# f1tenth/f1tenth_gym

Measured on AMD Instinct MI355X. Metric: agent-steps/s (1080-beam scan + ST dynamics), higher is better.
Workload: dtype f64

## Files before the change

f1tenth_gym_amd/csrc/f110_hip.hip:

```cpp
#include <hip/hip_runtime.h>
#include <rccl/rccl.h>

#include <dlfcn.h>

#include <algorithm>
#include <chrono>
#include <cmath>
#include <cstdarg>
#include <cstdio>
#include <cstdlib>
#include <cstring>
#include <map>
#include <mutex>
#include <new>
#include <set>
#include <string>
#include <vector>

#include "../../include/f110.h"
#include "f110_kernels.hpp"



#ifdef F110_EXPERIMENTAL
constexpr bool kExperimental = true;
#else
constexpr bool kExperimental = false;
#endif

struct ExpSwitches {
    int scan_flat = 0;
    int long_prio = 0;
    int scan_occupancy = 0;
    int scan_env_counter = 0;
    int integrate_duo = -1;
    int group_split = 0;
    int integrate_fan = -1;
    int tiny_general_tail = 0;
    int tiny_start_probe = 0;
    long probe_calls = 0;
    double probe_us[3] = {0, 0, 0};
    uint64_t tiny_trace = 0;
    uint64_t scan_trace = 0;
};

struct f110_sim {
    f110_config cfg{};
    int N = 0;
    hipStream_t stream = nullptr;
    hipStream_t side_stream = nullptr;
    hipEvent_t ev_integrated = nullptr, ev_collided = nullptr;
    AgentArrays dev{};
    ScanConst k{};
    bool has_map = false;
    uint32_t step_magic = 0, step_shift = 0;
    int scan_tasks_per_wave = 1, num_cus = 256;
    bool scan_tasks_auto = false;
    double ttc_side_max = INFINITY, ttc_cos_max = INFINITY;
    int dir_stride = 0;
    int scan_block = 64;
    double *d_params_all = nullptr;
    double *d_params = nullptr, *d_noise = nullptr, *d_scan_angles = nullptr, *d_beam_cos = nullptr, *d_side = nullptr;
    struct MapSlot {
        double *d_dt_row = nullptr, *d_dt_pad = nullptr;
        ScanConst k{};
        uint8_t *d_occ = nullptr;
    };
    std::vector<MapSlot> extra_maps;
    MapFast *d_maps_fast = nullptr;
    ScanConst *d_maps_full = nullptr;
    int32_t *d_env_map = nullptr;
    uint32_t *d_scan_order = nullptr;
    bool multi_map = false;
    ScanConst *d_k = nullptr;
    ScanConst k_uploaded{};
    unsigned long long *d_path_stats = nullptr;
    bool path_stats_on = false;
    double *d_dt_row = nullptr, *d_dt_pad = nullptr, *d_actions = nullptr, *d_poses = nullptr;
    double2 *d_cs = nullptr;
    uint8_t *d_mask = nullptr;
    int groups = 1;
    std::vector<hipStream_t> gstreams;
    std::vector<hipStream_t> gowned;
    std::vector<hipEvent_t> gevents;
    hipEvent_t ev_main = nullptr;
    bool groups_auto = true;
    bool touched = true;
    int last_blocks = 0;
    int group_probes = 0;
    bool groups_busy = false;
    bool main_dirty = true;
    NoiseGen noise_gen{};
    uint64_t *d_zig_k = nullptr;
    double *d_zig_w = nullptr, *d_zig_f = nullptr;
    U128 *d_jump = nullptr;
    U128 *d_rng_state = nullptr, *d_rng_seed = nullptr, *d_rng_rowstate = nullptr;
    int noise_rows_ready = 0;
    int noise_rows_alloc = 0;
    hipStream_t noise_stream = nullptr;
    hipEvent_t ev_noise = nullptr, ev_noise_src = nullptr;
    bool noise_ahead = false;
    int noise_ahead_upto = 0, noise_ahead_alloc = 0;
    double *noise_ahead_block = nullptr;
    std::vector<double *> noise_retired;
    long long noise_ub = 0;
    int noise_src = 0;
    uint64_t noise_src_id[4] = {0, 0, 0, 0};
    void *d_state_blob = nullptr;
    size_t state_blob_bytes = 0;
    unsigned long long *d_lookups = nullptr;
    bool lookups_on = false;
    int collide_mode = 0;
    bool task_order = false;
    uint32_t *d_tflags[2] = {nullptr, nullptr}, *d_tlist[2] = {nullptr, nullptr}, *d_tcount = nullptr;
    TaskSched tsched[2]{};
    bool sched_allocated = false;
    uint32_t task_cap_alloc = 0;
    uint32_t task_epoch = 2, task_cap = 0, task_thr = 96;
    uint32_t task_cap_div = 32, task_rev = 0;
    ExpSwitches exp;
    uint32_t *d_env_done = nullptr;
// ... 13 lines not shown
    EpisodeArrays ep{};
    bool has_episode = false;
    double *d_rot_stage = nullptr;
    void *d_packed = nullptr;
    bool hb_valid = false;
    f110_host_block hb_host{};
    HostBlock hb_dev{};
    const double *hb_actions_host = nullptr, *hb_actions_dev = nullptr;
    bool hb_scans_by_kernel = false;
    unsigned long long *hb_seq_host = nullptr;
    unsigned int *hb_blocks_done = nullptr;
    unsigned long long hb_seq = 0;
    double hs_enqueue_us = 0, hs_wait_us = 0;
    FusedHost *d_fused = nullptr;
    FusedHost fused_host_copy{};
    bool fused_valid = false;
    long long hs_calls = 0;
    TinyCtl tiny{};
    void *tiny_mem = nullptr;
    int tiny_off = 0;
    int last_launches = 0;
    struct TrackSlot {
        double *d_cols = nullptr;
        double *d_pts = nullptr;
        double *d_attr = nullptr;
        int32_t nattr = 0;
        int32_t nseg = 0, closed = 0, npts = 0;
        double L = 0.0;
    };
    std::vector<TrackSlot> tracks;
    TrackDesc *d_tracks = nullptr;
    PreviewAttr *d_track_attrs = nullptr;
    int n_tracks_dev = 0;
    bool tracks_dirty = true;
    bool track_lds = false;
    bool track_on = false, track_checked = false;
    std::vector<int32_t> env_map_host;
    double *d_trk = nullptr;
    int32_t *d_trk_seg = nullptr;
    double *d_trk_cache = nullptr;
    int32_t *d_trk_ok = nullptr;
    f110_track_host trk_pinned{};
    HostBlock trk_hb{};
    bool trk_pinned_on = false;
    const float *obs_pinned = nullptr;
    const float *preview_pinned = nullptr;
    const float *neighbors_pinned = nullptr;
    const float *rollout_pinned = nullptr;
    double *d_roll_end = nullptr;
    size_t roll_end_cap = 0;
    GapSpec *d_gap_specs = nullptr;
    int32_t *d_gap_assign = nullptr;
    int gap_specs = 0, gap_max_w = 0;
    uint8_t *d_occ0 = nullptr;
    std::vector<RenderSlot> render_slots;
    RenderSlot *d_render_slots = nullptr;
    size_t render_slots_cap = 0;
    RenderFrame *d_render_frames = nullptr;
    size_t render_frames_cap = 0;
    RenderCar *d_render_cars = nullptr;
    int32_t *d_render_agents = nullptr;
    size_t render_agents_cap = 0;
    uint8_t *d_render_stage = nullptr;
    size_t render_stage_cap = 0;
    struct ResetSampler {
        bool on = false;
        SamplerJob job{};
    } rs;
    hipEvent_t ev_begin = nullptr, ev_end = nullptr;
    bool profiling = false;
    std::vector<hipEvent_t> prof_events;
    size_t prof_used = 0;
    char err[512] = {0};
};

struct StepRequest {
    bool tiny = false;
    const double *tiny_actions = nullptr;
    bool fuse = false;
    unsigned long long seq = 0;
    const HostBlock *hb = nullptr;
    int episode = 0, auto_reset = 0;
    bool defer_draw = false;
};

static thread_local char g_err[512] = {0};

static int fail(f110_sim *h, int code, const char *fmt, ...)
{
    char buf[512];
    va_list ap;
    va_start(ap, fmt);
    vsnprintf(buf, sizeof buf, fmt, ap);
    va_end(ap);
    snprintf(g_err, sizeof g_err, "%s", buf);
    if (h) snprintf(h->err, sizeof h->err, "%s", buf);
    return code;
}

#define HIPCHK(h, call)                                                                              \
    do {                                                                                             \
        hipError_t e_ = (call);                                                                      \
        if (e_ != hipSuccess)                                                                        \
            return fail(h, F110_ERR_HIP, "%s failed: %s (%s:%d)", #call, hipGetErrorString(e_), __FILE__, __LINE__); \
    } while (0)

template <typename T>
static int dmalloc(f110_sim *h, T **p, size_t count)
{
    HIPCHK(h, hipMalloc(reinterpret_cast<void **>(p), count * sizeof(T) > 0 ? count * sizeof(T) : 8));
    return F110_OK;
}

#define TRY(expr)              \
    do {                       \
        int rc_ = (expr);      \
        if (rc_ != F110_OK) return rc_; \
    } while (0)

static int join_groups(f110_sim *h)
{
    if (h->comm_inflight) {
        HIPCHK(h, hipStreamWaitEvent(h->stream, h->ev_gather_done[0], 0));
        HIPCHK(h, hipStreamWaitEvent(h->stream, h->ev_gather_done[1], 0));
        h->comm_inflight = false;
    }
    if (!h->groups_busy) return F110_OK;
    for (size_t g = 0; g < h->gstreams.size(); ++g) {
        if (h->gstreams[g] == h->stream) continue;
        HIPCHK(h, hipEventRecord(h->gevents[g], h->gstreams[g]));
        HIPCHK(h, hipStreamWaitEvent(h->stream, h->gevents[g], 0));
    }
    h->groups_busy = false;
    return F110_OK;
}

#define ENTER(h)                                          \
    do {                                                  \
        HIPCHK(h, hipSetDevice((h)->cfg.device_id));      \
        TRY(join_groups(h));                              \
        (h)->main_dirty = true;                           \
        (h)->touched = true;                              \
    } while (0)

static int track_invalidate(f110_sim *h);
static int track_prepare(f110_sim *h);
static int track_launch(f110_sim *h, hipStream_t st, int mode, int begin, int count);
static bool tiny_applies(const f110_sim *h);
static void noise_release(f110_sim *h);
static void sampler_release(f110_sim *h);
static int sampler_launch(f110_sim *h, hipStream_t st, int mode, int e0, int count, const uint8_t *d_mask, int ego);
static int step_submit(f110_sim *h, const double *d_actions, const StepRequest &rq, bool &host_written);

constexpr int kMaxEnvBlocks = 16;
struct EnvBlock { hipStream_t stream; int e0, count; };
static void gap_launch_armed(f110_sim *h, const EnvBlock &b, double *d_actions);
struct EnvBlocks {
    EnvBlock b[kMaxEnvBlocks];
    int n = 0;
    const EnvBlock *begin() const { return b; }
    const EnvBlock *end() const { return b + n; }
};

static int group_envs(const f110_sim *h)
{
    const int E = h->cfg.num_envs, G = h->groups;
// ... 136 lines not shown
}

static int task_order_setup(f110_sim *h, bool on)
{
    const size_t n_tasks = (size_t)h->N * (((size_t)h->cfg.num_beams + 63) / 64);
    if (!on || n_tasks >= 0x7fffffffu) {
        h->task_order = false;
        return F110_OK;
    }
    if (!h->sched_allocated) {
        h->task_cap_alloc = (uint32_t)std::max<size_t>(64, kExperimental ? n_tasks : n_tasks / h->task_cap_div);
        for (int q = 0; q < 2; ++q) {
            TRY(dmalloc(h, &h->d_tflags[q], n_tasks));
            TRY(dmalloc(h, &h->d_tlist[q], (size_t)h->task_cap_alloc));
            HIPCHK(h, hipMemsetAsync(h->d_tflags[q], 0, sizeof(uint32_t) * n_tasks, h->stream));
        }
        TRY(dmalloc(h, &h->d_tcount, 4));
        HIPCHK(h, hipMemsetAsync(h->d_tcount, 0, 4 * sizeof(uint32_t), h->stream));
        h->sched_allocated = true;
    }
    h->task_cap = std::min<uint32_t>(h->task_cap_alloc, (uint32_t)std::max<size_t>(64, n_tasks / h->task_cap_div));
    for (int q = 0; q < 2; ++q)
        h->tsched[q] = TaskSched{h->d_tflags[q ^ 1], h->d_tflags[q], h->d_tlist[q ^ 1], h->d_tlist[q], h->d_tcount + (q ^ 1), h->d_tcount + q, h->task_cap, h->task_thr, {nullptr, nullptr, nullptr, nullptr, nullptr, nullptr, nullptr, nullptr}, 0u, 0u};
    HIPCHK(h, hipStreamSynchronize(h->stream));
    h->task_order = true;
    return F110_OK;
}

extern "C" {

const char *f110_last_error(const f110_sim *h) { return (h && h->err[0]) ? h->err : g_err; }
int f110_abi_version(void) { return F110_ABI_VERSION; }

int f110_device_count(int *count)
{
    int n = 0;
    hipError_t e = hipGetDeviceCount(&n);
    if (e != hipSuccess) {
        if (count) *count = 0;
        return fail(nullptr, F110_ERR_HIP, "hipGetDeviceCount failed: %s", hipGetErrorString(e));
    }
    if (count) *count = n;
    return F110_OK;
}

int f110_device_pci_bus_id(int32_t device, char *out, int32_t len)
{
    if (!out || len < 16) return fail(nullptr, F110_ERR_INVALID, "f110_device_pci_bus_id: buffer of at least 16 bytes required");
    const hipError_t e = hipDeviceGetPCIBusId(out, len, device);
    if (e != hipSuccess) return fail(nullptr, F110_ERR_HIP, "hipDeviceGetPCIBusId(%d) failed: %s", device, hipGetErrorString(e));
    return F110_OK;
}

#ifndef F110_SRC_HASH
#define F110_SRC_HASH "unknown"
#endif
const char *f110_build_info(void) { return "csrc=" F110_SRC_HASH; }

int f110_is_experimental(void) { return kExperimental ? 1 : 0; }

int f110_exp_set(f110_sim *h, const char *key, int32_t value)
{
    if (!h || !key) return fail(h, F110_ERR_INVALID, "null argument");
    if (!kExperimental) return fail(h, F110_ERR_STATE, "f110_exp_set(%s) is available in the experimental build only (libf110_hip_exp.so)", key);
    ENTER(h);
    HIPCHK(h, hipStreamSynchronize(h->stream));
    const std::string k(key);
    if (k == "scan_flat") h->exp.scan_flat = value;
    else if (k == "long_prio") h->exp.long_prio = value;
    else if (k == "scan_occupancy") h->exp.scan_occupancy = value;
    else if (k == "scan_env_counter") h->exp.scan_env_counter = value;
    else if (k == "integrate_duo") h->exp.integrate_duo = value;
    else if (k == "integrate_fan") h->exp.integrate_fan = value;
    else if (k == "group_split") h->exp.group_split = value;
    else if (k == "step_tiny") h->tiny_off = value == 0 ? 1 : 0;
    else if (k == "tiny_start_probe") {
        if (!value && h->exp.tiny_start_probe && h->exp.probe_calls)
            std::fprintf(stderr, "[tiny_start_probe] %ld steps: call -> launched %.2f us, launched -> first wave seen %.2f us, first wave seen -> completion word seen %.2f us\n",
                         h->exp.probe_calls, h->exp.probe_us[0] / h->exp.probe_calls, h->exp.probe_us[1] / h->exp.probe_calls, h->exp.probe_us[2] / h->exp.probe_calls);
        h->exp.tiny_start_probe = value;
        h->exp.probe_calls = 0;
        h->exp.probe_us[0] = h->exp.probe_us[1] = h->exp.probe_us[2] = 0;
    }
    else if (k == "tiny_general_tail") h->exp.tiny_general_tail = value;
    else if (k == "tiny_trace_hi") h->exp.tiny_trace = (h->exp.tiny_trace & 0xffffffffull) | ((uint64_t)(uint32_t)value << 32);
    else if (k == "tiny_trace_lo") h->exp.tiny_trace = (h->exp.tiny_trace & ~0xffffffffull) | (uint64_t)(uint32_t)value;
    else if (k == "scan_trace_hi") h->exp.scan_trace = (h->exp.scan_trace & 0xffffffffull) | ((uint64_t)(uint32_t)value << 32);
    else if (k == "scan_trace_lo") h->exp.scan_trace = (h->exp.scan_trace & ~0xffffffffull) | (uint64_t)(uint32_t)value;
    else if (k == "collide_mode") {
        if (value < 0 || value > 3) return fail(h, F110_ERR_INVALID, "collide_mode must be 0..3");
        h->collide_mode = value;
    }
    else if (k == "task_order") return task_order_setup(h, value != 0);
    else if (k == "task_cap_div" || k == "task_rev") {
        if (k == "task_rev") h->task_rev = value != 0;
        else h->task_cap_div = (uint32_t)std::max(1, value);
        if (h->task_order) return task_order_setup(h, true);
    } else if (k == "task_thr") {
        h->task_thr = (uint32_t)value;
        if (h->task_order) return task_order_setup(h, true);
    }
    else if (k == "pad_tiled" || k == "scan_nt" || k == "finalize_wave" || k == "spec_from" || k == "scan_stream" || k == "stream_refill" || k == "stream_block" ||
             k == "stream_grid")
        return fail(h, F110_ERR_INVALID, "f110_exp_set: '%s' was retired in round 6 with the variant it switched (DESIGN.md section 8)", key);
    else
        return fail(h, F110_ERR_INVALID, "f110_exp_set: unknown key '%s'", key);
    return F110_OK;
}

static void default_beam_tables(const f110_config &c, std::vector<double> &sa, std::vector<double> &co, std::vector<double> &sd)
{
    const int B = c.num_beams;
    const double incr = c.fov / (B - 1);
    const double dist_sides = c.params[F110_P_WIDTH] / 2., dist_fr = (c.params[F110_P_LF] + c.params[F110_P_LR]) / 2.;
    sa.resize(B); co.resize(B); sd.resize(B);
    for (int i = 0; i < B; ++i) {
        const double angle = -c.fov / 2. + i * incr;
        double to_side, to_fr;
        sa[i] = angle;
        co[i] = std::cos(angle);
        if (angle > 0) {
            if (angle < kPi / 2) { to_side = dist_sides / std::sin(angle); to_fr = dist_fr / std::cos(angle); }
            else { to_side = dist_sides / std::cos(angle - kPi / 2.); to_fr = dist_fr / std::sin(angle - kPi / 2.); }
        } else {
            if (angle > -kPi / 2) { to_side = dist_sides / std::sin(-angle); to_fr = dist_fr / std::cos(-angle); }
            else { to_side = dist_sides / std::cos(-angle - kPi / 2); to_fr = dist_fr / std::sin(-angle - kPi / 2); }
        }
        sd[i] = to_side < to_fr ? to_side : to_fr;
    }
}

static hipError_t streams_concurrent(hipStream_t a, hipStream_t b, bool *yes)
{
    *yes = false;
    unsigned *d = nullptr, hres[2] = {0u, 0u};
    hipError_t e = hipMalloc(&d, 2 * sizeof(unsigned));
    if (e != hipSuccess) return e;
    do {
        if ((e = hipMemsetAsync(d, 0, 2 * sizeof(unsigned), a)) != hipSuccess) break;
        if ((e = hipStreamSynchronize(a)) != hipSuccess) break;
        if ((e = hipStreamSynchronize(b)) != hipSuccess) break;
        hipLaunchKernelGGL(k_probe_wait, dim3(1), dim3(1), 0, a, d, d + 1, 30000ull);
        hipLaunchKernelGGL(k_probe_set, dim3(1), dim3(1), 0, b, d);
        if ((e = hipStreamSynchronize(a)) != hipSuccess) break;
        if ((e = hipStreamSynchronize(b)) != hipSuccess) break;
        if ((e = hipMemcpy(hres, d, sizeof hres, hipMemcpyDeviceToHost)) != hipSuccess) break;
        *yes = hres[1] != 0u;
    } while (0);
    (void)hipFree(d);
    return e;
}

static std::mutex g_registry_mu;
static std::set<f110_sim *> g_handles;
static std::map<const char *, size_t> g_host_blocks;

int f110_create(const f110_config *cfg, f110_sim **out)
{
    if (!cfg || !out) return fail(nullptr, F110_ERR_INVALID, "f110_create: null argument");
    *out = nullptr;
    if (cfg->abi_version != F110_ABI_VERSION) return fail(nullptr, F110_ERR_INVALID, "ABI version mismatch (%d vs %d)", cfg->abi_version, F110_ABI_VERSION);
    if (cfg->num_envs < 1 || cfg->num_agents < 1 || cfg->num_beams < 2 || cfg->theta_dis < 2)
        return fail(nullptr, F110_ERR_INVALID, "f110_create: num_envs/num_agents >= 1, num_beams/theta_dis >= 2 required");
    if (cfg->integrator != F110_INTEGRATOR_RK4 && cfg->integrator != F110_INTEGRATOR_EULER)
        return fail(nullptr, F110_ERR_INVALID, "Invalid Integrator Specified. Please choose RK4 or Euler");
    if (cfg->map_layout == F110_MAP_TILED_F64 || cfg->map_layout == F110_MAP_CODE8 || cfg->map_layout == F110_MAP_WINDOW_LDS)
// ... 1958 lines not shown
#define DIRS_SCAN(PM, ID)                                                                                                                    \
    do {                                                                                                                                     \
        if (cnt) hipLaunchKernelGGL((k_scan_dirs_agent<PM, ID, true>), grid, block, 0, st, j, h->k, h->d_maps_fast, h->d_maps_full, tpa);     \
        else hipLaunchKernelGGL((k_scan_dirs_agent<PM, ID, false>), grid, block, 0, st, j, h->k, h->d_maps_fast, h->d_maps_full, tpa);        \
    } while (0)
            if (h->multi_map) DIRS_SCAN(true, false);
            else if (h->k.ident_rot) DIRS_SCAN(false, true);
            else DIRS_SCAN(false, false);
#undef DIRS_SCAN
            break;
        }
        case SCAN_AGENT_SCHED: {
            const uint32_t tpa = ((uint32_t)B + 63u) / 64u;
            agent_grid(tpa, grid, wpb, h->scan_tasks_per_wave);
            const uint32_t parity = h->task_epoch & 1u;
            j.sched = h->tsched[parity];
            j.epoch_r = h->task_epoch - 1u;
            j.epoch_w = h->task_epoch;
            j.long_blocks = (h->task_cap + wpb - 1) / wpb;
            j.long_prio = (uint32_t)h->exp.long_prio;
            j.long_rev = h->task_rev;
            h->task_epoch += 1u;
            const dim3 sgrid(grid.x + j.long_blocks);
            size_t slds = 0;
#ifdef F110_EXPERIMENTAL
            if (h->exp.scan_occupancy > 0 && h->scan_block == 64) slds = (size_t)(160 * 1024 / (4 * h->exp.scan_occupancy)) & ~(size_t)255;
#endif
            if (h->k.ident_rot)
                hipLaunchKernelGGL((k_scan_rays_agent<false, true, false, true>), sgrid, block, slds, st, j, h->k, h->d_maps_fast, h->d_maps_full, tpa);
            else
                hipLaunchKernelGGL((k_scan_rays_agent<false, false, false, true>), sgrid, block, slds, st, j, h->k, h->d_maps_fast, h->d_maps_full, tpa);
            break;
        }
        case SCAN_AGENT: {
            const uint32_t tpa = ((uint32_t)B + 63u) / 64u;
            agent_grid(tpa, grid, wpb, h->scan_tasks_per_wave);
            size_t lds = 0;
#ifdef F110_EXPERIMENTAL
            if (h->exp.scan_occupancy > 0 && h->scan_block == 64) lds = (size_t)(160 * 1024 / (4 * h->exp.scan_occupancy)) & ~(size_t)255;
            if (h->exp.scan_env_counter && !h->multi_map && !cnt) {
                if (!h->d_env_done) {
                    TRY(dmalloc(h, &h->d_env_done, (size_t)h->cfg.num_envs));
                    HIPCHK(h, hipMemsetAsync(h->d_env_done, 0, sizeof(uint32_t) * h->cfg.num_envs, st));
                }
                j.env_done = h->d_env_done;
                j.tasks_per_env = tpa * (uint32_t)A;
                if (h->k.ident_rot)
                    hipLaunchKernelGGL((k_scan_rays_agent<false, true, false, false, true>), grid, block, lds, st, j, h->k, h->d_maps_fast, h->d_maps_full, tpa);
                else
                    hipLaunchKernelGGL((k_scan_rays_agent<false, false, false, false, true>), grid, block, lds, st, j, h->k, h->d_maps_fast, h->d_maps_full, tpa);
                break;
            }
#endif
#define AGENT_SCAN(PM, ID)                                                                                                           \
    do {                                                                                                                             \
        if (cnt)                                                                                                                     \
            hipLaunchKernelGGL((k_scan_rays_agent<PM, ID, true>), grid, block, lds, st, j, h->k, h->d_maps_fast, h->d_maps_full, tpa); \
        else                                                                                                                         \
            hipLaunchKernelGGL((k_scan_rays_agent<PM, ID, false>), grid, block, lds, st, j, h->k, h->d_maps_fast, h->d_maps_full, tpa); \
    } while (0)
            if (h->multi_map)
                AGENT_SCAN(true, false);
            else if (h->k.ident_rot)
                AGENT_SCAN(false, true);
            else
                AGENT_SCAN(false, false);
#undef AGENT_SCAN
            break;
        }
        default: {
            const dim3 fgrid = rays_grid(j, h->scan_block, h->scan_tasks_per_wave);
            hipLaunchKernelGGL(pick_rays<true>(h->k, h->cfg.map_layout), fgrid, block, 0, st, j, h->k);
            break;
        }
        }
    }
    if (ev) HIPCHK(h, hipEventRecord(ev[2], st));
    if (side_collide) HIPCHK(h, hipStreamWaitEvent(st, h->ev_collided, 0));
    if (multi) {
        const bool narrow = h->dev.reseat_poses != nullptr;
        int lanes = narrow && N >= 131072 ? 8 : (narrow && N >= (pair_in_finalize ? 8192 : 32768) ? 16 : 64);
        if (pair_in_finalize) {
            lanes = N >= 32768 ? 8 : (N >= 4096 ? 16 : 64);
            if (rq.fuse && begin == 0 && count == N && !dev.reseat_poses) {
                dev.fused_host = h->d_fused;
                dev.fused_seq = rq.seq;
                host_written = true;
            }
            if (dev.fused_host) {
                if (lanes <= 8) hipLaunchKernelGGL((k_finalize_pair_roles<32, true>), dim3((count + 31) / 32), dim3(256), 0, st, dev, B);
                else if (lanes == 16) hipLaunchKernelGGL((k_finalize_pair_roles<16, true>), dim3((count + 15) / 16), dim3(256), 0, st, dev, B);
                else hipLaunchKernelGGL((k_finalize_pair_roles<4, true>), dim3((count + 3) / 4), dim3(256), 0, st, dev, B);
            } else if (lanes <= 8) hipLaunchKernelGGL(k_finalize_pair_roles<32>, dim3((count + 31) / 32), dim3(256), 0, st, dev, B);
            else if (lanes == 16) hipLaunchKernelGGL(k_finalize_pair_roles<16>, dim3((count + 15) / 16), dim3(256), 0, st, dev, B);
            else hipLaunchKernelGGL(k_finalize_pair_roles<4>, dim3((count + 3) / 4), dim3(256), 0, st, dev, B);
        }
        else if (multi_in_finalize) {
            const int envs = count / A;
            if (A * (A - 1) <= kMaxRec) {
                const int G = kMaxRec / (A * (A - 1));
                hipLaunchKernelGGL(k_finalize_multi<kMaxRec>, dim3((envs + G - 1) / G), dim3(256), 0, st, dev, B, G);
            } else if (A * (A - 1) <= kMaxRecBig) {
                hipLaunchKernelGGL(k_finalize_multi<kMaxRecBig>, dim3(envs), dim3(256), 0, st, dev, B, 1);
            } else {
                hipLaunchKernelGGL(k_finalize_multi_tiled<kMaxRecBig>, dim3(envs), dim3(256), multi_lds_bytes(A, kMaxRecBig), st, dev, B, 1);
            }
        }
        else if (lanes == 8)
            hipLaunchKernelGGL(k_finalize<8>, dim3((count + 31) / 32), dim3(256), 0, st, dev, B);
        else if (lanes == 16)
            hipLaunchKernelGGL(k_finalize<16>, dim3((count + 15) / 16), dim3(256), 0, st, dev, B);
        else
            hipLaunchKernelGGL(k_finalize<64>, dim3((count + 3) / 4), dim3(256), 0, st, dev, B);
    } else {
        hipLaunchKernelGGL(k_finalize_solo, grid1d(count, 256), dim3(256), 0, st, dev);
    }
    if (ev) HIPCHK(h, hipEventRecord(ev[3], st));
    if (h->track_on) TRY(track_launch(h, st, kTrackPost, begin, count));
    return F110_OK;
}

static bool env_blocks_pay(int N, int A)
{
    if (A == 2 && N > 32768) return false;
    if (A <= 4 && N >= 2560 && N <= 5120) return false;
    return true;
}

int f110_step_groups(f110_sim *h, int32_t *groups, int32_t *probes, int32_t *last)
{
    if (!h) return fail(h, F110_ERR_INVALID, "null argument");
    if (groups) *groups = h->groups;
    if (probes) *probes = h->group_probes;
    if (last) *last = h->last_blocks;
    return F110_OK;
}

int f110_step_launches(f110_sim *h, int32_t *launches)
{
    if (!h || !launches) return fail(h, F110_ERR_INVALID, "null argument");
    *launches = h->last_launches;
    return F110_OK;
}

static int step_submit(f110_sim *h, const double *d_actions, const StepRequest &rq, bool &host_written)
{
    host_written = false;
    HIPCHK(h, hipSetDevice(h->cfg.device_id));
    if (h->track_on || h->rs.on) TRY(track_prepare(h));
    const int N = h->N, A = h->cfg.num_agents;
    h->dev.path_stats = h->path_stats_on ? h->d_path_stats : nullptr;
    if (h->comm_overlap && h->comm_swap_next) {
        h->scans_cur ^= 1;
        h->dev.scans = h->scan_bufs[h->scans_cur];
        if (h->gather_pending[h->scans_cur]) {
            const bool inflight = h->comm_inflight;
            h->comm_inflight = false;
            const int rj = join_groups(h);
            h->comm_inflight = inflight;
            if (rj != F110_OK) return rj;
            HIPCHK(h, hipStreamWaitEvent(h->stream, h->ev_gather_done[h->scans_cur], 0));
            h->gather_pending[h->scans_cur] = false;
            h->main_dirty = true;
        }
        h->comm_swap_next = false;
    }
    if (h->dev.noise_rng == 1 && h->noise_rows_ready < h->dev.noise_rows) {
        if (h->noise_ub >= h->noise_rows_ready) {
            TRY(join_groups(h));
            TRY(noise_adopt(h));
            if (h->noise_ub >= h->noise_rows_ready && h->noise_rows_ready < h->dev.noise_rows) {
                const long long want = std::max<long long>(2LL * h->noise_rows_ready, h->noise_ub + 1);
                TRY(noise_cache_extend(h, (int)std::min<long long>(want, h->dev.noise_rows)));
            }
        }
        if (!h->noise_ahead && 2 * (h->noise_ub + 1) >= h->noise_rows_ready) TRY(noise_start_ahead(h));
    }
    const bool prof = h->profiling && h->prof_used + 4 <= 4 * 65536;
    const bool tiny = rq.tiny && !prof;
    const bool grouped = !tiny && h->groups > 1 && !prof && (h->multi_map || agent_aligned(h)) && h->dir_stride == 0 &&
                         !(h->gstreams[0] == h->stream && h->collide_mode != 3 && A > 1) &&
                         (!h->groups_auto || (!h->touched && env_blocks_pay(N, A)));
    h->last_launches = 0;
    const EnvBlocks w = grouped ? env_blocks_submit(h) : env_blocks_main(h);
    if (!grouped) {
        TRY(join_groups(h));
        h->main_dirty = true;
        hipEvent_t ev[4] = {nullptr, nullptr, nullptr, nullptr};
        if (prof) {
            for (int i = 0; i < 4; ++i)
                if (!(ev[i] = prof_event(h))) return fail(h, F110_ERR_HIP, "hipEventCreate failed");
        }
        if (tiny) TRY(step_tiny(h, h->stream, d_actions, rq, host_written));
        else TRY(step_range(h, h->stream, 0, N, d_actions, h->collide_mode, prof ? ev : nullptr, rq, host_written));
    } else {
        if (h->main_dirty) {
            HIPCHK(h, hipEventRecord(h->ev_main, h->stream));
            for (hipStream_t gs : h->gstreams)
                if (gs != h->stream) HIPCHK(h, hipStreamWaitEvent(gs, h->ev_main, 0));
            h->main_dirty = false;
        }
        const int mode = h->collide_mode == 3 ? 3 : ((A == 2 || A == 4) ? 1 : 2);
        for (const EnvBlock &b : w) TRY(step_range(h, b.stream, b.e0 * A, b.count * A, d_actions, mode, nullptr, rq, host_written));
        h->groups_busy = true;
    }
    if (h->rs.on && h->dev.reseat_poses && !rq.defer_draw) TRY(sampler_after_step(h, w));
    h->touched = false;
    h->last_blocks = grouped ? h->groups : 1;
    h->noise_ub += 1;
    HIPCHK(h, hipGetLastError());
    return F110_OK;
}

int f110_step_device(f110_sim *h, const double *d_actions)
{
    TRY(check_step(h, d_actions != nullptr));
    bool host_written = false;
    return step_submit(h, d_actions, StepRequest{}, host_written);
}

int f110_stream_fence(f110_sim *h)
{
    if (!h) return fail(nullptr, F110_ERR_INVALID, "null handle");
    ENTER(h);
    return F110_OK;
}

int f110_step(f110_sim *h, const double *actions)
{
    TRY(check_step(h, actions != nullptr));
    ENTER(h);
    HIPCHK(h, hipMemcpyAsync(h->d_actions, actions, sizeof(double) * 2 * h->N, hipMemcpyHostToDevice, h->stream));
    TRY(f110_step_device(h, h->d_actions));
    HIPCHK(h, hipStreamSynchronize(h->stream));
    return F110_OK;
}

static int copy_col(f110_sim *h, double *dst, const double *src, size_t n)
{
    if (dst) HIPCHK(h, hipMemcpyAsync(dst, src, n * sizeof(double), hipMemcpyDeviceToHost, h->stream));
    return F110_OK;
}

int f110_get_obs(f110_sim *h, const f110_obs_host *o)
{
    if (!h || !o) return fail(h, F110_ERR_INVALID, "null argument");
    ENTER(h);
    const size_t N = (size_t)h->N;
    const AgentArrays &d = h->dev;
    TRY(copy_col(h, o->scans, d.scans, N * h->cfg.num_beams));
    TRY(copy_col(h, o->poses_x, d.state, N));
    TRY(copy_col(h, o->poses_y, d.state + N, N));
    TRY(copy_col(h, o->poses_theta, d.state + 4 * N, N));
    TRY(copy_col(h, o->linear_vels_x, d.state + 3 * N, N));
    TRY(copy_col(h, o->ang_vels_z, d.state + 5 * N, N));
    TRY(copy_col(h, o->collisions, d.collisions, N));
    TRY(copy_col(h, o->collision_idx, d.collision_idx, N));
    std::vector<double> soa, poses;
    if (o->state) {
        soa.resize(7 * N);
        HIPCHK(h, hipMemcpyAsync(soa.data(), d.state, 7 * N * sizeof(double), hipMemcpyDeviceToHost, h->stream));
    }
    if (o->agent_poses) {
        poses.resize(3 * N);
        HIPCHK(h, hipMemcpyAsync(poses.data(), d.snap_pose, 3 * N * sizeof(double), hipMemcpyDeviceToHost, h->stream));
    }
    if (o->in_collision) HIPCHK(h, hipMemcpyAsync(o->in_collision, d.in_collision, N * sizeof(int32_t), hipMemcpyDeviceToHost, h->stream));
    if (o->step_count) HIPCHK(h, hipMemcpyAsync(o->step_count, d.step_count, N * sizeof(int32_t), hipMemcpyDeviceToHost, h->stream));
    HIPCHK(h, hipStreamSynchronize(h->stream));
    if (o->state)
        for (size_t i = 0; i < N; ++i)
            for (int c = 0; c < 7; ++c) o->state[7 * i + c] = soa[(size_t)c * N + i];
    if (o->agent_poses)
        for (size_t i = 0; i < N; ++i)
            for (int c = 0; c < 3; ++c) o->agent_poses[3 * i + c] = poses[(size_t)c * N + i];
    return F110_OK;
}

int f110_set_state(f110_sim *h, const double *state7, const double *steer_buf, const int32_t *buf_count)
{
    if (!h || !state7) return fail(h, F110_ERR_INVALID, "null argument");
    ENTER(h);
    const size_t N = (size_t)h->N;
    std::vector<double> soa(7 * N);
    for (size_t i = 0; i < N; ++i)
        for (int c = 0; c < 7; ++c) soa[(size_t)c * N + i] = state7[7 * i + c];
// ... 2075 lines not shown
```

f1tenth_gym_amd/csrc/f110_kernels.hpp:

```cpp
#pragma once

#include <hip/hip_runtime.h>
#include <stdint.h>

#include "f110_math.hpp"
#include "f110_rng.hpp"

using namespace f110;

struct RayHdr {
    double x, y;
    double start;
    double vel;
    double d0;
    int32_t noise_row;
    int32_t map_slot;
    int32_t pad_hdr;
    int32_t i0;
    int32_t n_dirs;
    int32_t fast;
};
static_assert(sizeof(RayHdr) == 64, "RayHdr is read as 16-byte scalar loads");

struct AgentArrays {
// ... 1349 lines not shown
                    d_rec[slot][1] = ey;
                    d_rec[slot][2] = eth;
#pragma unroll
                    for (int c = 0; c < 8; ++c) d_rec[slot][3 + c] = v[c];
                }
            } else {
                int cl, ch;
                disc_beam_range_from(norm, eth, dir, head, 0.5 * sqrt(blen * blen + bwid * bwid), a.scan_angles, B, a.angle_inc, cl, ch);
                d_cl[slot] = cl;
                d_ch[slot] = ch;
            }
        }
    }
    __syncthreads();
    const bool agent_thread = t < N;
    const int my_hit = d_hit;
    if (agent_thread) {
        const int i = t, me = i & 1;
        const int wall = a.in_collision[i];
        if (wall) {
            a.state[3 * (size_t)N + i] = 0.;
            a.state[4 * (size_t)N + i] = 0.;
            a.state[5 * (size_t)N + i] = 0.;
            a.state[6 * (size_t)N + i] = 0.;
        }
        a.collisions[i] = (my_hit || wall) ? 1.0 : 0.0;
        a.collision_idx[i] = my_hit ? (double)(1 - me) : -1.0;
        a.step_count[i] += 1;
    }
    {
        const int ag = t >> 7, tt = t & 127;
        const int i0 = d_idx[ag][0], i1 = d_idx[ag][1], i2 = d_idx[ag][2], i3 = d_idx[ag][3];
        const int cl = d_cl[ag], ch = d_ch[ag];
        int ref_lo = i0 < i1 ? i0 : i1, t2 = i2 < i3 ? i2 : i3;
        ref_lo = ref_lo < t2 ? ref_lo : t2;
        int ref_hi = i0 > i1 ? i0 : i1;
        t2 = i2 > i3 ? i2 : i3;
        ref_hi = ref_hi > t2 ? ref_hi : t2;
        const int lo = ref_lo > cl ? ref_lo : cl;
        const int hi = ref_hi < ch ? ref_hi : ch;
        const int cnt = hi >= lo ? hi - lo + 1 : 0;
        const double bex = d_rec[ag][0], bey = d_rec[ag][1], beth = d_rec[ag][2];
        double bv[8];
#pragma unroll
        for (int c = 0; c < 8; ++c) bv[c] = d_rec[ag][3 + c];
        double *sc = a.scans + (size_t)ag * B;
        for (int item = tt; item < cnt; item += 128) {
            const int b = lo + item;
            const double bt = beth + a.scan_angles[b];
            const double r0 = sc[b];
            double v3x, v3y;
            sincos(bt + kPi / 2., &v3y, &v3x);
            const double r = box_range(bex, bey, v3x, v3y, bv, r0);
            if (r < r0) {
                sc[b] = r;
                if (HOST && host_scans) host_scans[(size_t)ag * B + b] = r;
            }
        }
    }
    if (HOST) {
        if (fh.hb.scans && !host_scans) {
            __syncthreads();
            host_block_copy_scans(fh.hb, a.scans, 0, (size_t)N);
        }
        if (t < 64) pair_host_epilogue_with(a, fh.ep, fh.hb, fh.episode, fh.auto_reset, agent_thread, t);
    } else if (a.reseat_poses && agent_thread) {
        const int i = t, ego = a.reseat_ego;
        if (my_hit || a.in_collision[ego] != 0) reseat_agent(a, i, i == ego);
    }
}

#ifndef F110_FIN_WAVES
#define F110_FIN_WAVES 5
#endif
template <int AG, bool HOST = false>
__global__ void __launch_bounds__(256) __attribute__((amdgpu_waves_per_eu(HOST ? 4 : F110_FIN_WAVES))) k_finalize_pair_roles(AgentArrays a, int32_t B)
{
    finalize_pair_body<AG, HOST>(a, B, a.agent_begin + (int)blockIdx.x * AG, a.agent_begin + a.agent_count);
    if (HOST && a.fused_seq) {
        HostBlock sig = a.fused_host->hb;
        sig.seq = a.fused_seq;
        host_block_signal(sig);
    }
}

constexpr int kMaxRec = 64;
constexpr int kMaxRecBig = 256;
constexpr int kMultiCornerThreads = 192;
struct MultiAgentLds {
    double ex, ey, eth, head;
    double ox, oy, co, so;
    double blen, bwid, rad;
};
template <int MAXREC>
__global__ void __launch_bounds__(256) k_finalize_multi(AgentArrays a, int32_t B, int G)
{
    static_assert(MAXREC == 64 || MAXREC == 256, "record table sizes");
    __shared__ double s_rec[MAXREC][12];
    __shared__ int s_idx[MAXREC][4], s_cl[MAXREC], s_ch[MAXREC], s_hit[MAXREC];
    __shared__ int s_lo[MAXREC], s_off[MAXREC + 1], s_agent[MAXREC], s_ahit[MAXREC], s_wsum[4];
    constexpr int MAXAG = MAXREC == 64 ? 32 : 16;
    __shared__ MultiAgentLds s_ag[MAXAG];
    const int t = (int)threadIdx.x;
    const int A = a.agents_per_env, N = a.n_agents_total;
    const int per_env = A * (A - 1), pairs_env = per_env / 2;
    const int first = a.agent_begin + (int)blockIdx.x * G * A, end = a.agent_begin + a.agent_count;
    int envs = (end - first) / A;
    envs = envs < G ? envs : G;
    const int R = envs * per_env, P = envs * pairs_env, AGN = envs * A;
    if (t < AGN) {
        const int i = first + t;
        MultiAgentLds m;
        m.ex = a.state[i];
        m.ey = a.state[(size_t)N + i];
        const double th_live = a.state[4 * (size_t)N + i];
        m.eth = a.in_collision[i] ? 0.0 : th_live;
        double ce_, se_;
        cos_sin(m.eth, ce_, se_);
        m.head = atan2(se_, ce_);
        m.ox = a.snap_pose[i];
        m.oy = a.snap_pose[(size_t)N + i];
        cos_sin(a.snap_pose[2 * (size_t)N + i], m.co, m.so);
        const size_t prow = (size_t)(a.params_per_agent ? i : t % A) * NPARAMS;
        m.blen = a.params[prow + P_LENGTH];
        m.bwid = a.params[prow + P_WIDTH];
        m.rad = 0.5 * sqrt(m.blen * m.blen + m.bwid * m.bwid);
        s_ag[t] = m;
    }
    __syncthreads();
    if (t < kMultiCornerThreads) {
        for (int q = t; q < 4 * R; q += kMultiCornerThreads) {
            const int rec = q >> 2, sub = q & 3;
            const int e = rec / per_env, w = rec - e * per_env, me = w / (A - 1), k = w - me * (A - 1), oj = k < me ? k : k + 1;
            const MultiAgentLds &mm = s_ag[e * A + me], &mo = s_ag[e * A + oj];
            const double ex = mm.ex, ey = mm.ey, eth = mm.eth, head = mm.head;
            double v[8];
            box_vertices_cs(mo.ox, mo.oy, mo.co, mo.so, mm.blen, mm.bwid, v);
            const double px = sub == 0 ? v[0] : (sub == 1 ? v[2] : (sub == 2 ? v[4] : v[6]));
            const double py = sub == 0 ? v[1] : (sub == 1 ? v[3] : (sub == 2 ? v[5] : v[7]));
            const double dx = px - ex, dy = py - ey;
            const double norm = sqrt(dx * dx + dy * dy);
            const double dir = atan2(dy / norm, dx / norm);
            s_idx[rec][sub] = vertex_beam_from_angles(head, dir, a.scan_angles, B, a.angle_inc);
            if (sub == 0) {
                s_rec[rec][0] = ex;
                s_rec[rec][1] = ey;
                s_rec[rec][2] = eth;
#pragma unroll
                for (int c = 0; c < 8; ++c) s_rec[rec][3 + c] = v[c];
                s_agent[rec] = e * A + me;
            }
        }
    } else {
        for (int rec = t - kMultiCornerThreads; rec < R; rec += 256 - kMultiCornerThreads) {
            const int e = rec / per_env, w = rec - e * per_env, me = w / (A - 1), k = w - me * (A - 1), oj = k < me ? k : k + 1;
            const MultiAgentLds &mm = s_ag[e * A + me], &mo = s_ag[e * A + oj];
            const double eth = mm.eth, head = mm.head;
            const double dx = mo.ox - mm.ex, dy = mo.oy - mm.ey;
            const double norm = sqrt(dx * dx + dy * dy);
            const double dir = atan2(dy, dx);
            int cl, ch;
            disc_beam_range_from(norm, eth, dir, head, mm.rad, a.scan_angles, B, a.angle_inc, cl, ch);
            s_cl[rec] = cl;
            s_ch[rec] = ch;
        }
        const double reach = sqrt(a.box_length * a.box_length + a.box_width * a.box_width) + 1e-3;
// ... 2520 lines not shown
```

f1tenth_gym_amd/csrc/f110_math.hpp:

```cpp
#pragma once

#include <hip/hip_runtime.h>
#include <math.h>
#include <stdint.h>

#define F110_HD __host__ __device__ __forceinline__

namespace f110 {

constexpr double kPi = 3.14159265358979323846;
constexpr double kTwoPi = 2.0 * kPi;

enum { P_MU = 0, P_CSF, P_CSR, P_LF, P_LR, P_H, P_M, P_I, P_SMIN, P_SMAX, P_SVMIN, P_SVMAX,
       P_VSWITCH, P_AMAX, P_VMIN, P_VMAX, P_WIDTH, P_LENGTH, NPARAMS };

struct VehicleParams {
    double v[NPARAMS];
};

F110_HD void cos_sin(double a, double &c, double &s)
{
#if defined(__HIP_DEVICE_COMPILE__)
    sincos(a, &s, &c);
#else
// ... 683 lines not shown
F110_HD int vertex_beam_from_angles(double head, double dir, const double *scan_angles, int num_beams, double angle_inc)
{
    double angle = head - dir;
    if (angle > kPi)
        angle = angle - 2 * kPi;
    else if (angle < -kPi)
        angle = angle + 2 * kPi;
    return nearest_beam(scan_angles, num_beams, angle_inc, -angle);
}

F110_HD int vertex_beam_index(double ex, double ey, double etheta, double vx, double vy,
                              const double *scan_angles, int num_beams, double angle_inc)
{
    const double dx = vx - ex, dy = vy - ey;
    const double norm = sqrt(dx * dx + dy * dy);
    const double ux = dx / norm, uy = dy / norm;
    double ce, se;
    cos_sin(etheta, ce, se);
    return vertex_beam_from_angles(atan2(se, ce), atan2(uy, ux), scan_angles, num_beams, angle_inc);
}

F110_HD void disc_beam_range_from(double dist, double eth, double dir, double head, double R, const double *scan_angles, int num_beams,
                                  double angle_inc, int &cl, int &ch)
{
    if (!(dist > R * 1.000001 + 1e-9) || !(fabs(eth) < 1e6)) {
        cl = 0;
        ch = num_beams - 1;
        return;
    }
    double phi = dir - head;
    phi -= kTwoPi * rint(phi / kTwoPi);
    const double psi = asin(R / dist) + 3.0 * angle_inc + 1e-6;
    const double sa0 = scan_angles[0];
    const double last = (double)(num_beams - 1);
    cl = num_beams;
    ch = -1;
#pragma unroll
    for (int k = -1; k <= 1; ++k) {
        double lo = ceil((phi + kTwoPi * k - psi - sa0) / angle_inc);
        double hi = floor((phi + kTwoPi * k + psi - sa0) / angle_inc);
        lo = lo < 0.0 ? 0.0 : lo;
        hi = hi > last ? last : hi;
        if (lo <= hi) {
            cl = (int)lo < cl ? (int)lo : cl;
            ch = (int)hi > ch ? (int)hi : ch;
        }
    }
}

F110_HD void disc_beam_range(double ex, double ey, double eth, double cx, double cy, double R,
                             const double *scan_angles, int num_beams, double angle_inc, int &cl, int &ch)
{
    const double dx = cx - ex, dy = cy - ey;
    const double dist = sqrt(dx * dx + dy * dy);
    if (!(dist > R * 1.000001 + 1e-9) || !(fabs(eth) < 1e6)) {
        cl = 0;
        ch = num_beams - 1;
        return;
    }
    double ce, se;
    cos_sin(eth, ce, se);
    disc_beam_range_from(dist, eth, atan2(dy, dx), atan2(se, ce), R, scan_angles, num_beams, angle_inc, cl, ch);
}

F110_HD void opponent_beam_window(double ex, double ey, double eth, const double *v, double cx, double cy,
                                  double R, const double *scan_angles, int num_beams, double angle_inc,
                                  int &ref_lo, int &ref_hi, int &lo, int &hi)
{
    const int i0 = vertex_beam_index(ex, ey, eth, v[0], v[1], scan_angles, num_beams, angle_inc);
    const int i1 = vertex_beam_index(ex, ey, eth, v[2], v[3], scan_angles, num_beams, angle_inc);
    const int i2 = vertex_beam_index(ex, ey, eth, v[4], v[5], scan_angles, num_beams, angle_inc);
    const int i3 = vertex_beam_index(ex, ey, eth, v[6], v[7], scan_angles, num_beams, angle_inc);
    int a = i0 < i1 ? i0 : i1, b = i2 < i3 ? i2 : i3;
    ref_lo = a < b ? a : b;
    a = i0 > i1 ? i0 : i1;
    b = i2 > i3 ? i2 : i3;
    ref_hi = a > b ? a : b;
    int cl, ch;
    disc_beam_range(ex, ey, eth, cx, cy, R, scan_angles, num_beams, angle_inc, cl, ch);
    lo = ref_lo > cl ? ref_lo : cl;
    hi = ref_hi < ch ? ref_hi : ch;
}

F110_HD double box_range(double ex, double ey, double v3x, double v3y, const double *v, double r)
{
    double rr = edge_range(ex, ey, v3x, v3y, v[0], v[1], v[2], v[3]);
    if (rr < r) r = rr;
    rr = edge_range(ex, ey, v3x, v3y, v[2], v[3], v[4], v[5]);
    if (rr < r) r = rr;
    rr = edge_range(ex, ey, v3x, v3y, v[4], v[5], v[6], v[7]);
    if (rr < r) r = rr;
    rr = edge_range(ex, ey, v3x, v3y, v[6], v[7], v[0], v[1]);
    if (rr < r) r = rr;
    return r;
}

F110_HD void box_vertices(double x, double y, double th, double length, double width, double *v)
{
    double c, s;
    cos_sin(th, c, s);
    const double hx = length / 2, hy = width / 2;
    const double bx[4] = {-hx, -hx, hx, hx};
    const double by[4] = {hy, -hy, -hy, hy};
#pragma unroll
    for (int i = 0; i < 4; ++i) {
        v[2 * i] = ((c * bx[i] + (-s) * by[i]) + 0.) + x;
        v[2 * i + 1] = ((s * bx[i] + c * by[i]) + 0.) + y;
    }
}

F110_HD void box_vertices_cs(double x, double y, double c, double s, double length, double width, double *v)
{
    const double hx = length / 2, hy = width / 2;
    const double bx[4] = {-hx, -hx, hx, hx};
    const double by[4] = {hy, -hy, -hy, hy};
#pragma unroll
    for (int i = 0; i < 4; ++i) {
        v[2 * i] = ((c * bx[i] + (-s) * by[i]) + 0.) + x;
        v[2 * i + 1] = ((s * bx[i] + c * by[i]) + 0.) + y;
    }
}

F110_HD int furthest_vertex(const double *v, double dx, double dy)
{
    int best = 0;
    double bv = v[0] * dx + v[1] * dy;
#pragma unroll
    for (int i = 1; i < 4; ++i) {
        const double val = v[2 * i] * dx + v[2 * i + 1] * dy;
        if (val > bv) {
            bv = val;
            best = i;
        }
    }
    return best;
}

F110_HD void minkowski_support(const double *v1, const double *v2, double dx, double dy, double &ax, double &ay)
{
    const int i = furthest_vertex(v1, dx, dy);
    const int j = furthest_vertex(v2, -dx, -dy);
    ax = v1[2 * i] - v2[2 * j];
    ay = v1[2 * i + 1] - v2[2 * j + 1];
}

F110_HD void triple_product(double ax, double ay, double bx, double by, double cx, double cy, double &ox, double &oy)
{
    const double ac = ax * cx + ay * cy;
    const double bc = bx * cx + by * cy;
    ox = bx * ac - ax * bc;
    oy = by * ac - ay * bc;
}

F110_HD bool gjk_overlap(const double *v1, const double *v2)
{
    double s0x, s0y, s1x = 0, s1y = 0;
    double dx = (((v1[0] + v1[2]) + v1[4]) + v1[6]) / 4 - (((v2[0] + v2[2]) + v2[4]) + v2[6]) / 4;
    double dy = (((v1[1] + v1[3]) + v1[5]) + v1[7]) / 4 - (((v2[1] + v2[3]) + v2[5]) + v2[7]) / 4;
    if (dx == 0 && dy == 0) dx = 1.0;
    double ax, ay;
    minkowski_support(v1, v2, dx, dy, ax, ay);
    s0x = ax;
    s0y = ay;
    if (dx * ax + dy * ay <= 0) return false;
    dx = -ax;
    dy = -ay;
    int index = 0;
    for (int iter = 0; iter < 1000;) {
        minkowski_support(v1, v2, dx, dy, ax, ay);
        index += 1;
        if (dx * ax + dy * ay <= 0) return false;
        const double aox = -ax, aoy = -ay;
        if (index < 2) {
            s1x = ax;
            s1y = ay;
            const double abx = s0x - ax, aby = s0y - ay;
            triple_product(abx, aby, aox, aoy, abx, aby, dx, dy);
            if (sqrt(dx * dx + dy * dy) < 1e-10) {
                dx = aby;
                dy = -1 * abx;
            }
            continue;
        }
        const double abx = s1x - ax, aby = s1y - ay;
        const double acx = s0x - ax, acy = s0y - ay;
        double px, py;
        triple_product(abx, aby, acx, acy, acx, acy, px, py);
        if (px * aox + py * aoy >= 0) {
            dx = px;
            dy = py;
        } else {
            triple_product(acx, acy, abx, aby, abx, aby, px, py);
            if (px * aox + py * aoy < 0) return true;
            s0x = s1x;
            s0y = s1y;
            dx = px;
            dy = py;
        }
        s1x = ax;
        s1y = ay;
        index -= 1;
        ++iter;
    }
    return false;
}


F110_HD int nearest_on_trajectory(const double *wp, int M, double px, double py, double &dist, double &t_best)
{
    int best = 0;
    dist = INFINITY;
    t_best = 0.0;
    for (int k = 0; k + 1 < M; ++k) {
        const double ax = wp[3 * k], ay = wp[3 * k + 1];
        const double dx = wp[3 * k + 3] - ax, dy = wp[3 * k + 4] - ay;
        double t = ((px - ax) * dx + (py - ay) * dy) / (dx * dx + dy * dy);
        t = t < 0.0 ? 0.0 : (t > 1.0 ? 1.0 : t);
        const double rx = px - (ax + t * dx), ry = py - (ay + t * dy);
        const double d = sqrt(rx * rx + ry * ry);
        if (d < dist) {
            dist = d;
            t_best = t;
            best = k;
        }
    }
    return best;
}

F110_HD bool lookahead_cuts(double sx, double sy, double ex, double ey, double px, double py, double radius, double t_min)
{
    const double vx = (ex + 1e-6) - sx, vy = (ey + 1e-6) - sy;
    const double a = vx * vx + vy * vy;
    const double b = 2.0 * (vx * (sx - px) + vy * (sy - py));
    const double c = (sx * sx + sy * sy) + (px * px + py * py) - 2.0 * (sx * px + sy * py) - radius * radius;
    const double disc = b * b - 4 * a * c;
    if (disc < 0) return false;
    const double root = sqrt(disc);
    const double t1 = (-b - root) / (2.0 * a), t2 = (-b + root) / (2.0 * a);
    return (t1 >= 0.0 && t1 <= 1.0 && t1 >= t_min) || (t2 >= 0.0 && t2 <= 1.0 && t2 >= t_min);
}

F110_HD int first_waypoint_on_circle(const double *wp, int M, double px, double py, double radius, double start)
{
    const int start_i = (int)start;
    const double start_t = fmod(start, 1.0);
    for (int i = start_i; i + 1 < M; ++i)
        if (lookahead_cuts(wp[3 * i], wp[3 * i + 1], wp[3 * i + 3], wp[3 * i + 4], px, py, radius, i == start_i ? start_t : 0.0))
            return i;
    for (int i = -1; i < start_i; ++i) {
        const int k0 = i < 0 ? M - 1 : i, k1 = i + 1;
        if (lookahead_cuts(wp[3 * k0], wp[3 * k0 + 1], wp[3 * k1], wp[3 * k1 + 1], px, py, radius, 0.0)) return k0;
    }
    return -1;
}

F110_HD void pure_pursuit_plan(const double *wp, int M, double px, double py, double theta, double lookahead, double vgain,
                               double wheelbase, double max_reacquire, double &steer, double &speed)
{
    steer = 0.0;
    speed = 4.0;
    double dist, t;
    const int i = nearest_on_trajectory(wp, M, px, py, dist, t);
    int goal = i;
    if (dist < lookahead) {
        goal = first_waypoint_on_circle(wp, M, px, py, lookahead, (double)i + t);
        if (goal < 0) return;
    } else if (!(dist < max_reacquire)) {
        return;
    }
    const double wy = sin(-theta) * (wp[3 * goal] - px) + cos(-theta) * (wp[3 * goal + 1] - py);
    speed = vgain * wp[3 * i + 2];
    if (fabs(wy) < 1e-6) return;
    const double radius = 1 / (2.0 * wy / (lookahead * lookahead));
    steer = atan(wheelbase / radius);
}

constexpr int kObsFeatures = 8;
enum { OBS_POOL_MIN = 0, OBS_POOL_MEAN = 1, OBS_POOL_CENTER = 2 };

struct ObsRowSpec {
    int32_t W, K;
    int32_t pool, D;
    int32_t nfeat;
    int32_t feat[kObsFeatures];
    double clip, scale;
    double feat_scale[kObsFeatures];
};

F110_HD double obs_minimum(double v, double clip) { return v != v ? v : (v < clip ? v : clip); }
// ... 555 lines not shown
```

Measured before the change: 95.71 million.

## Add single-wave pair finalize kernel for env-block steps

Result: faster. 102.2 million (median of 6 runs) (+6.7%).

```diff
diff --git a/f1tenth_gym_amd/csrc/f110_hip.hip b/f1tenth_gym_amd/csrc/f110_hip.hip
--- a/f1tenth_gym_amd/csrc/f110_hip.hip
+++ b/f1tenth_gym_amd/csrc/f110_hip.hip
@@ -37,6 +37,7 @@
     int group_split = 0;
     int integrate_fan = -1;
     int tiny_general_tail = 0;
+    int pair_wave = -1;
     int tiny_start_probe = 0;
     long probe_calls = 0;
     double probe_us[3] = {0, 0, 0};
@@ -216,6 +217,7 @@
     const HostBlock *hb = nullptr;
     int episode = 0, auto_reset = 0;
     bool defer_draw = false;
+    bool env_blocks = false;
 };
 
 static thread_local char g_err[512] = {0};
@@ -518,6 +520,7 @@
         h->exp.probe_calls = 0;
         h->exp.probe_us[0] = h->exp.probe_us[1] = h->exp.probe_us[2] = 0;
     }
+    else if (k == "pair_wave") h->exp.pair_wave = value;
     else if (k == "tiny_general_tail") h->exp.tiny_general_tail = value;
     else if (k == "tiny_trace_hi") h->exp.tiny_trace = (h->exp.tiny_trace & 0xffffffffull) | ((uint64_t)(uint32_t)value << 32);
     else if (k == "tiny_trace_lo") h->exp.tiny_trace = (h->exp.tiny_trace & ~0xffffffffull) | (uint64_t)(uint32_t)value;
@@ -2642,6 +2645,10 @@
         int lanes = narrow && N >= 131072 ? 8 : (narrow && N >= (pair_in_finalize ? 8192 : 32768) ? 16 : 64);
         if (pair_in_finalize) {
             lanes = N >= 32768 ? 8 : (N >= 4096 ? 16 : 64);
+            bool pair_wave = rq.env_blocks && (!h->groups_auto || N >= 24576);
+#ifdef F110_EXPERIMENTAL
+            if (h->exp.pair_wave >= 0) pair_wave = h->exp.pair_wave != 0;
+#endif
             if (rq.fuse && begin == 0 && count == N && !dev.reseat_poses) {
                 dev.fused_host = h->d_fused;
                 dev.fused_seq = rq.seq;
@@ -2651,6 +2658,9 @@
                 if (lanes <= 8) hipLaunchKernelGGL((k_finalize_pair_roles<32, true>), dim3((count + 31) / 32), dim3(256), 0, st, dev, B);
                 else if (lanes == 16) hipLaunchKernelGGL((k_finalize_pair_roles<16, true>), dim3((count + 15) / 16), dim3(256), 0, st, dev, B);
                 else hipLaunchKernelGGL((k_finalize_pair_roles<4, true>), dim3((count + 3) / 4), dim3(256), 0, st, dev, B);
+            } else if (pair_wave) {
+                constexpr int AG = kFinalizeWaveAgents;
+                hipLaunchKernelGGL(k_finalize_pair_wave<AG>, dim3((count + AG - 1) / AG), dim3(64), 0, st, dev, B);
             } else if (lanes <= 8) hipLaunchKernelGGL(k_finalize_pair_roles<32>, dim3((count + 31) / 32), dim3(256), 0, st, dev, B);
             else if (lanes == 16) hipLaunchKernelGGL(k_finalize_pair_roles<16>, dim3((count + 15) / 16), dim3(256), 0, st, dev, B);
             else hipLaunchKernelGGL(k_finalize_pair_roles<4>, dim3((count + 3) / 4), dim3(256), 0, st, dev, B);
@@ -2682,7 +2692,6 @@
 
 static bool env_blocks_pay(int N, int A)
 {
-    if (A == 2 && N > 32768) return false;
     if (A <= 4 && N >= 2560 && N <= 5120) return false;
     return true;
 }
@@ -2761,7 +2770,9 @@
             h->main_dirty = false;
         }
         const int mode = h->collide_mode == 3 ? 3 : ((A == 2 || A == 4) ? 1 : 2);
-        for (const EnvBlock &b : w) TRY(step_range(h, b.stream, b.e0 * A, b.count * A, d_actions, mode, nullptr, rq, host_written));
+        StepRequest rb = rq;
+        rb.env_blocks = true;
+        for (const EnvBlock &b : w) TRY(step_range(h, b.stream, b.e0 * A, b.count * A, d_actions, mode, nullptr, rb, host_written));
         h->groups_busy = true;
     }
     if (h->rs.on && h->dev.reseat_poses && !rq.defer_draw) TRY(sampler_after_step(h, w));
diff --git a/f1tenth_gym_amd/csrc/f110_kernels.hpp b/f1tenth_gym_amd/csrc/f110_kernels.hpp
--- a/f1tenth_gym_amd/csrc/f110_kernels.hpp
+++ b/f1tenth_gym_amd/csrc/f110_kernels.hpp
@@ -1455,6 +1455,149 @@
         sig.seq = a.fused_seq;
         host_block_signal(sig);
     }
+}
+
+template <int AG>
+__device__ __forceinline__ void finalize_pair_wave_body(const AgentArrays &a, int32_t B, const int first, const int end)
+{
+    constexpr int NT = 64;
+    constexpr int AGP = AG <= 2 ? 2 : (AG <= 4 ? 4 : (AG <= 8 ? 8 : 16));
+    static_assert(AG >= 2 && (AG & 1) == 0 && 5 * AG <= NT && AG <= AGP, "whole envs, and 4 AG corner + AG cull lanes fit the wave");
+    constexpr int R1 = 4 * AG;
+    typedef const volatile __attribute__((address_space(3))) double *LdsBox;
+    __shared__ double s_rec[AG][12];
+    __shared__ int s_idx[AG][4], s_cl[AG], s_ch[AG], s_hit[AG / 2];
+    __shared__ int s_lo[AG], s_cnt[AG], s_off[AGP + 1];
+    __shared__ double s_box[AG / 2][16];
+    __shared__ int s_ab[NT][2];
+    const int t = (int)threadIdx.x;
+    const int N = a.n_agents_total;
+    const int role = t < R1 ? 0 : (t < R1 + AG ? 1 : -1);
+    const int slot = role == 0 ? t >> 2 : t - R1, sub = t & 3;
+    bool near = false;
+    if (role >= 0 && first + slot < end) {
+        const int i = first + slot, me = i & 1, o = i ^ 1;
+        const double ex = a.state[i], ey = a.state[(size_t)N + i];
+        const double th_live = a.state[4 * (size_t)N + i];
+        const double ox = a.snap_pose[o], oy = a.snap_pose[(size_t)N + o], oth = a.snap_pose[2 * (size_t)N + o];
+        const int wall = a.in_collision[i];
+        const double eth = wall ? 0.0 : th_live;
+        const size_t prow = (size_t)(a.params_per_agent ? i : me) * NPARAMS;
+        const double blen = a.params[prow + P_LENGTH], bwid = a.params[prow + P_WIDTH];
+        double v[8];
+        box_vertices(ox, oy, oth, blen, bwid, v);
+        double ce_, se_;
+        cos_sin(eth, ce_, se_);
+        const double head = atan2(se_, ce_);
+        const double px = role == 1 ? ox : (sub == 0 ? v[0] : (sub == 1 ? v[2] : (sub == 2 ? v[4] : v[6])));
+        const double py = role == 1 ? oy : (sub == 0 ? v[1] : (sub == 1 ? v[3] : (sub == 2 ? v[5] : v[7])));
+        const double dx = px - ex, dy = py - ey;
+        const double d2 = dx * dx + dy * dy;
+        const double norm = sqrt(d2);
+        const double qx = role == 0 ? dx / norm : dx, qy = role == 0 ? dy / norm : dy;
+        const double dir = atan2(qy, qx);
+        if (role == 0) {
+            s_idx[slot][sub] = vertex_beam_from_angles(head, dir, a.scan_angles, B, a.angle_inc);
+            if (sub == 0) {
+                s_rec[slot][0] = ex;
+                s_rec[slot][1] = ey;
+                s_rec[slot][2] = eth;
+#pragma unroll
+                for (int c = 0; c < 8; ++c) s_rec[slot][3 + c] = v[c];
+            }
+        } else {
+            int cl, ch;
+            disc_beam_range_from(norm, eth, dir, head, 0.5 * sqrt(blen * blen + bwid * bwid), a.scan_angles, B, a.angle_inc, cl, ch);
+            s_cl[slot] = cl;
+            s_ch[slot] = ch;
+            const double reach = sqrt(a.box_length * a.box_length + a.box_width * a.box_width) + 1e-3;
+            near = me == 0 && d2 <= reach * reach;
+        }
+    }
+    int hit = 0;
+    if (__ballot(near) != 0) {
+        if (near) {
+            const int i = first + slot, o = i ^ 1;
+            double *mine = s_box[slot >> 1], *other = mine + 8;
+            box_vertices(a.state[i], a.state[(size_t)N + i], a.state[4 * (size_t)N + i], a.box_length, a.box_width, mine);
+            box_vertices(a.snap_pose[o], a.snap_pose[(size_t)N + o], a.snap_pose[2 * (size_t)N + o], a.box_length, a.box_width, other);
+            hit = gjk_overlap_from<LdsBox>((LdsBox)mine, (LdsBox)other) ? 1 : 0;
+        }
+    }
+    if (role == 1 && (slot & 1) == 0) s_hit[slot >> 1] = hit;
+    __syncthreads();
+    if (t < AG) {
+        int lo = 0, cnt = 0;
+        if (first + t < end) {
+            const int i = first + t, me = i & 1;
+            const int i0 = s_idx[t][0], i1 = s_idx[t][1], i2 = s_idx[t][2], i3 = s_idx[t][3];
+            const int cl = s_cl[t], ch = s_ch[t];
+            const int my_hit = s_hit[t >> 1];
+            int ref_lo = i0 < i1 ? i0 : i1, t2 = i2 < i3 ? i2 : i3;
+            ref_lo = ref_lo < t2 ? ref_lo : t2;
+            int ref_hi = i0 > i1 ? i0 : i1;
+            t2 = i2 > i3 ? i2 : i3;
+            ref_hi = ref_hi > t2 ? ref_hi : t2;
+            lo = ref_lo > cl ? ref_lo : cl;
+            const int hi = ref_hi < ch ? ref_hi : ch;
+            cnt = hi >= lo ? hi - lo + 1 : 0;
+            const int wall = a.in_collision[i];
+            if (wall) {
+                a.state[3 * (size_t)N + i] = 0.;
+                a.state[4 * (size_t)N + i] = 0.;
+                a.state[5 * (size_t)N + i] = 0.;
+                a.state[6 * (size_t)N + i] = 0.;
+            }
+            a.collisions[i] = (my_hit || wall) ? 1.0 : 0.0;
+            a.collision_idx[i] = my_hit ? (double)(1 - me) : -1.0;
+            a.step_count[i] += 1;
+        }
+        s_lo[t] = lo;
+        s_cnt[t] = cnt;
+    }
+    __syncthreads();
+    {
+        int c = t < AG ? s_cnt[t] : 0;
+#pragma unroll
+        for (int d = 1; d < AGP; d <<= 1) {
+            const int up = __shfl_up(c, d);
+            if (t >= d) c += up;
+        }
+        if (t < AGP) s_off[t + 1] = c;
+        if (t == 0) s_off[0] = 0;
+    }
+    __syncthreads();
+    for (int item = t; item < s_off[AG]; item += NT) {
+        int ag = 0;
+#pragma unroll
+        for (int st = AGP / 2; st; st >>= 1)
+            if (s_off[ag + st] <= item) ag += st;
+        int b = s_lo[ag] + (item - s_off[ag]);
+        const double bt = s_rec[ag][2] + a.scan_angles[b];
+        s_ab[item & (NT - 1)][0] = ag;
+        s_ab[item & (NT - 1)][1] = b;
+        double v3x, v3y;
+        sincos(bt + kPi / 2., &v3y, &v3x);
+        __asm__ volatile("" ::: "memory");
+        ag = s_ab[item & (NT - 1)][0];
+        b = s_ab[item & (NT - 1)][1];
+        double *sc = a.scans + (size_t)(first + ag) * B;
+        const double r0 = sc[b];
+        const double r = box_range_from<LdsBox>(s_rec[ag][0], s_rec[ag][1], v3x, v3y, (LdsBox)&s_rec[ag][3], r0);
+        if (r < r0) sc[b] = r;
+    }
+    const int te = (int)__builtin_amdgcn_mbcnt_hi(~0u, __builtin_amdgcn_mbcnt_lo(~0u, 0u));
+    if (a.reseat_poses && te < AG && first + te < end) {
+        const int i = first + te, ego = (i & ~1) + a.reseat_ego;
+        if (s_hit[te >> 1] || a.in_collision[ego] != 0) reseat_agent(a, i, i == ego);
+    }
+}
+
+constexpr int kFinalizeWaveAgents = 12;
+template <int AG>
+__global__ void __launch_bounds__(64) __attribute__((amdgpu_waves_per_eu(8))) k_finalize_pair_wave(AgentArrays a, int32_t B)
+{
+    finalize_pair_wave_body<AG>(a, B, a.agent_begin + (int)blockIdx.x * AG, a.agent_begin + a.agent_count);
 }
 
 constexpr int kMaxRec = 64;
diff --git a/f1tenth_gym_amd/csrc/f110_math.hpp b/f1tenth_gym_amd/csrc/f110_math.hpp
--- a/f1tenth_gym_amd/csrc/f110_math.hpp
+++ b/f1tenth_gym_amd/csrc/f110_math.hpp
@@ -789,7 +789,8 @@
     hi = ref_hi < ch ? ref_hi : ch;
 }
 
-F110_HD double box_range(double ex, double ey, double v3x, double v3y, const double *v, double r)
+template <typename V>
+F110_HD double box_range_from(double ex, double ey, double v3x, double v3y, V v, double r)
 {
     double rr = edge_range(ex, ey, v3x, v3y, v[0], v[1], v[2], v[3]);
     if (rr < r) r = rr;
@@ -802,6 +803,11 @@
     return r;
 }
 
+F110_HD double box_range(double ex, double ey, double v3x, double v3y, const double *v, double r)
+{
+    return box_range_from<const double *>(ex, ey, v3x, v3y, v, r);
+}
+
 F110_HD void box_vertices(double x, double y, double th, double length, double width, double *v)
 {
     double c, s;
@@ -828,7 +834,8 @@
     }
 }
 
-F110_HD int furthest_vertex(const double *v, double dx, double dy)
+template <typename V>
+F110_HD int furthest_vertex(V v, double dx, double dy)
 {
     int best = 0;
     double bv = v[0] * dx + v[1] * dy;
@@ -843,7 +850,8 @@
     return best;
 }
 
-F110_HD void minkowski_support(const double *v1, const double *v2, double dx, double dy, double &ax, double &ay)
+template <typename V>
+F110_HD void minkowski_support(V v1, V v2, double dx, double dy, double &ax, double &ay)
 {
     const int i = furthest_vertex(v1, dx, dy);
     const int j = furthest_vertex(v2, -dx, -dy);
@@ -859,7 +867,8 @@
     oy = by * ac - ay * bc;
 }
 
-F110_HD bool gjk_overlap(const double *v1, const double *v2)
+template <typename V>
+F110_HD bool gjk_overlap_from(V v1, V v2)
 {
     double s0x, s0y, s1x = 0, s1y = 0;
     double dx = (((v1[0] + v1[2]) + v1[4]) + v1[6]) / 4 - (((v2[0] + v2[2]) + v2[4]) + v2[6]) / 4;
@@ -912,6 +921,8 @@
     return false;
 }
 
+F110_HD bool gjk_overlap(const double *v1, const double *v2) { return gjk_overlap_from<const double *>(v1, v2); }
+
 
 F110_HD int nearest_on_trajectory(const double *wp, int M, double px, double py, double &dist, double &t_best)
 {
```
